# Victarry/Image-Generation-models

Measured on AMD Instinct MI355X. Metric: ddpm_cifar10_32x32_train_images_per_sec, higher is better.
Workload: dtype bf16; 1 GPU; DDPM CIFAR-10 32x32, UNet 128/1-2-4, T=1000 (BASELINE configs[1]): train step B=128/GPU + hipGraph denoise step B=64; per_gpu_batch=128, global_batch=128, parallelism=dp1, step_launch=hipGraph replay, denoise_batch=64, rccl_ranks=1, state_finite=True, matmul=bf16 MFMA, fp32 accumulate

## Files before the change

image-generation-models_amd/csrc/conv_pw.hip:

```cpp
#include "tr_common.h"

#ifndef MI_PW_PABL
#define MI_PW_PABL 0
#endif
#ifndef MI_PW_GNSABL
#define MI_PW_GNSABL 0
#endif
#ifndef MI_PW_FXABL
#define MI_PW_FXABL 0
#endif
#ifdef MI_PW_TIMING
__device__ uint32_t g_pw_ts[1024 * 4 * 5 * 64];
__device__ __forceinline__ uint32_t pw_wlane(uint32_t val, uint32_t lane, uint32_t v) {
    uint32_t keep;
    asm volatile("s_mov_b32 %1, m0\n\ts_mov_b32 m0, %3\n\ts_nop 0\n\tv_writelane_b32 %0, %2, m0\n\ts_mov_b32 m0, %1"
                 : "+v"(v), "=&s"(keep) : "s"(__builtin_amdgcn_readfirstlane(val)), "s"(__builtin_amdgcn_readfirstlane(lane)));
    return v;
}
extern "C" int mi_debug_pw_ts(uint32_t* host_out) { return (int)hipMemcpyFromSymbol(host_out, HIP_SYMBOL(g_pw_ts), sizeof(g_pw_ts)); }
#endif

namespace {

typedef uint32_t u32x2 __attribute__((ext_vector_type(2)));
// ... 1 lines not shown
__device__ __attribute__((aligned(16))) uint32_t g_zero_page3[64];

struct PwArgs {
    const uint16_t* x; const uint16_t* x2; const uint16_t* w; const float* bias; const float* res; void* y;
    int N, H, W, K, Nc, K1, ldx, ldx2, ldy, ldr, accumulate, flip;
    int TH, TI, XP, tiles_per_img, xmap;
    int qmap, gx, gy;
    uint32_t tpi_magic, cpq_magic, nch_magic, cpg_magic; int ppx, cpq, lnsub;
    const void* zero;
    float* gsum;
    const float* coef;
    const float* sums; const float* gamma; const float* beta; const float* temb;
    int ldt, cpg, hw, ng; float eps;
    double icnt;
    int ksplit; float* sk_part; int* sk_flag;
};

constexpr int pw_xp(int pt) { return pt == 256 ? 320 : pt == 128 ? 192 : 128; }

__device__ __forceinline__ int pw_fastdiv(int x, uint32_t magic) { return magic ? (int)__umulhi((uint32_t)x, magic) : x; }
inline uint32_t pw_magic(int d) { return d > 1 ? (uint32_t)((0x100000000ULL + (unsigned)d - 1) / (unsigned)d) : 0u; }

__device__ __forceinline__ void glds16s(const void* sbase, uint32_t voff, uint32_t lds_dst) {
    const uint64_t p = (uint64_t)(uintptr_t)sbase;
    const uint32_t lo = __builtin_amdgcn_readfirstlane((uint32_t)p), hi = __builtin_amdgcn_readfirstlane((uint32_t)(p >> 32));
    const uint64_t q = ((uint64_t)hi << 32) | lo;
    const uint32_t dst = __builtin_amdgcn_readfirstlane(lds_dst);
    uint32_t keep;
    asm volatile("s_mov_b32 %0, m0\n\ts_mov_b32 m0, %3\n\ts_nop 0\n\tglobal_load_lds_dwordx4 %1, %2\n\ts_mov_b32 m0, %0"
                 : "=&s"(keep) : "v"(voff), "s"(q), "s"(dst) : "memory");
// ... 31 lines not shown
    const u32x4 v = __builtin_bit_cast(u32x4, c);
    uint32_t a0, a1;
    if constexpr (DIR == 0)
        asm("v_and_b32_dpp %0, %2, %4 wave_shr:1 row_mask:0xf bank_mask:0xf bound_ctrl:1\n\t"
            "v_and_b32_dpp %1, %3, %4 wave_shr:1 row_mask:0xf bank_mask:0xf bound_ctrl:1"
            : "=&v"(a0), "=&v"(a1) : "v"(v[2 * HALF]), "v"(v[2 * HALF + 1]), "v"(mask));
    else
        asm("v_and_b32_dpp %0, %2, %4 wave_shl:1 row_mask:0xf bank_mask:0xf bound_ctrl:1\n\t"
            "v_and_b32_dpp %1, %3, %4 wave_shl:1 row_mask:0xf bank_mask:0xf bound_ctrl:1"
            : "=&v"(a0), "=&v"(a1) : "v"(v[2 * HALF]), "v"(v[2 * HALF + 1]), "v"(mask));
    o[2 * HALF] = a0; o[2 * HALF + 1] = a1;
}

constexpr int pw_lds(int pt, bool raw = false) { return (pt == 256 ? 128 : pt == 128 ? (raw ? 72 : 64) : (raw ? 48 : 32)) * 1024 + 2048; }

template <bool OUT16, int VAR = 0, int ZERO = 0, int PT = 128, bool IN32 = false, bool F32 = false>
__global__ __launch_bounds__(256, PT == 256 ? 1 : 2) void conv_pw_kernel(const PwArgs a) {
    MI_PRIO_UP();
    static_assert(ZERO == 0, "unused: kept so that the recorded kernel symbols (profiles, launch-name tests) stay valid");
#ifdef MI_PW_TIMING
    constexpr bool TIMED = VAR == 0 && !IN32 && !F32;
    uint32_t tv[5] = {0u, 0u, 0u, 0u, 0u};
    uint64_t tprev = 0;
    if constexpr (TIMED) {
        tprev = __builtin_amdgcn_s_memtime();
        tv[4] = pw_wlane((uint32_t)wall_clock64(), 7, tv[4]);
        tv[4] = pw_wlane((uint32_t)tprev, 3, tv[4]);
    }
#define MI_PW_STAMP(SET, LANE) do { if constexpr (TIMED) { tv[SET] = pw_wlane((uint32_t)tprev, (LANE), tv[SET]); tprev = __builtin_amdgcn_s_memtime(); } } while (0)
#define MI_PW_NOW(LANE) do { if constexpr (TIMED) { tv[4] = pw_wlane((uint32_t)__builtin_amdgcn_s_memtime(), (LANE), tv[4]); } } while (0)
#else
#define MI_PW_STAMP(SET, LANE) do {} while (0)
#define MI_PW_NOW(LANE) do {} while (0)
#endif
// ... 749 lines not shown
                for (int rq = 0; rq < 4; ++rq) {
                    const int ck = 8 * wv + 2 * rq + (l >> 5);
                    typedef __attribute__((address_space(3))) f32x4 lds_f32x4b;
                    const f32x4 bq = *(lds_f32x4b*)(uintptr_t)(lds0 + BIASL + 16 * ck);
#pragma unroll
                    for (int i = 0; i < BH; ++i) {
                        const int p = ep_p0 + i * a.W;
                        *(lds_u32x2*)(uintptr_t)(lds0 + p * 256 + ((ck ^ ((p & 15) << 1)) << 3)) =
                            u32x2{pack_bf16(acc[i][4 * rq] + bq.x, acc[i][4 * rq + 1] + bq.y), pack_bf16(acc[i][4 * rq + 2] + bq.z, acc[i][4 * rq + 3] + bq.w)};
                    }
                }
            }
            __syncthreads();
            MI_PW_NOW(14);
            const int j = t & 15, col = n0 + 8 * j;
            float gs[2][2] = {{0.f, 0.f}, {0.f, 0.f}};
            if (col < a.Nc) {
#pragma unroll
                for (int it = 0; it < PT / 16; ++it) {
                    const int p = it * 16 + (t >> 4);
                    const u32x4 o = *(lds_u32x4e*)(uintptr_t)(lds0 + p * 256 + (((2 * j) ^ ((p & 15) << 1)) << 3));
                    *reinterpret_cast<u32x4*>(reinterpret_cast<uint16_t*>(a.y) + ((size_t)m0 + p) * a.ldy + col) = o;
                    if constexpr (GNS && MI_PW_GNSABL != 2) {
#pragma unroll
                        for (int q = 0; q < 4; ++q) {
                            const float e0 = __uint_as_float(o[q] << 16), e1 = __uint_as_float(o[q] & 0xffff0000u);
                            gs[PT >= 256 ? 0 : it / (PT / 32)][0] += e0 + e1; gs[PT >= 256 ? 0 : it / (PT / 32)][1] += e0 * e0 + e1 * e1;
                        }
                    }
                }
// ... 819 lines not shown
        if (d->K % 128 || d->K1 % 128 || d->K1 <= 0 || d->K1 > d->K || d->Nc % 64 || d->ldx % 4 || (d->K1 != d->K && d->ldx2 % 4)) return false;
        return ((long)d->N * d->OH * d->OW) % 128 == 0;
    }
    if (f32) {
        if (d->KH != 1 || d->KW != 1 || d->pad != 0 || d->stride != 1 || d->mode != 0 || d->IH != d->OH || d->IW != d->OW) return false;
        if (d->K % 64 || d->K1 % 64 || d->K1 <= 0 || d->K1 > d->K || d->Nc % 64 || d->ldx % 4 || (d->K1 != d->K && d->ldx2 % 4)) return false;
        return ((long)d->N * d->OH * d->OW) % 128 == 0;
    }
    if (d->KH != 1 || d->KW != 1 || d->pad != 0 || d->stride != 1 || d->mode != 1) return false;
    if (d->IH != d->OH || d->IW != d->OW) return false;
    if (d->K % 128 || d->K1 % 128 || d->K1 <= 0 || d->K1 > d->K || d->Nc % 64 || d->ldx % 8 || (d->K1 != d->K && d->ldx2 % 8)) return false;
    return ((long)d->N * d->OH * d->OW) % 128 == 0;
}

struct PwGn { const float* sums; const float* gamma; const float* beta; const float* temb; int ldt, G; float eps; };

static int pw_launch(const char* who, const MiConvDesc* d, const void* x, const void* x2, const void* w_frag_bf16, const float* bias,
                     const float* residual, void* y, int out_bf16, int var, float* gsum, const float* coef, void* stream,
                     const PwGn* gn = nullptr, bool in32 = false, bool f32 = false) {
    PwArgs a{};
    if (!d || !x || !w_frag_bf16 || !y) return mi_set_error(-1, "%s: null argument", who);
    const int pt = pw_pick_tile(d, var, &a.TH, &a.TI, in32, f32, &a.ksplit);
    if (!pt) return mi_set_error(-1, "%s: descriptor not supported by the private-weight-stream conv kernel", who);
    int dev_ = 0;
    (void)hipGetDevice(&dev_);
    if (a.ksplit > 1) {
        uint8_t* ws = reinterpret_cast<uint8_t*>(g_pw_sk_ws[dev_ & 63].load(std::memory_order_acquire));
        a.sk_flag = reinterpret_cast<int*>(ws); a.sk_part = reinterpret_cast<float*>(ws + PW_SK_FLAG_BYTES);
#ifdef MI_PW_SK_ABL
        a.sk_flag = nullptr;
#endif
    }
    if (d->K1 != d->K && !x2) return mi_set_error(-1, "%s: two-source split without x2", who);
    if ((((uintptr_t)x | (uintptr_t)(x2 ? x2 : x) | (uintptr_t)w_frag_bf16) & 15) != 0) return mi_set_error(-1, "%s: operands must be 16-byte aligned", who);
    if (d->ldy % 8 || (residual && d->ldr % 4)) return mi_set_error(-1, "%s: output pixel stride must be a multiple of 8, the residual's of 4", who);
    if (var >= 2 && (a.TI != 1 || d->K1 != d->K))
        return mi_set_error(-1, "%s: the fused variants need one image per tile and one source", who);
    if (var == 2 && (!coef || ((uintptr_t)coef & 15)))
// ... 31 lines not shown
    grid.z = (unsigned)a.ksplit;
    hipStream_t st = (hipStream_t)stream;
    size_t lds = pw_lds(pt, in32 && var < 2);
    if (var >= 2) {
        const size_t need = (size_t)2 * pw_xp(pt) * 128 + 2048 + (size_t)12 * d->K;
        if (need > lds) lds = need;
    }
#define MI_PW_GO_T(O16, V, T) do { \
        static MiPerDevice once_; \
        once_.run([] { (void)hipFuncSetAttribute((const void*)conv_pw_kernel<O16, V, 0, T>, hipFuncAttributeMaxDynamicSharedMemorySize, 160 * 1024); }); \
        hipLaunchKernelGGL((conv_pw_kernel<O16, V, 0, T>), grid, dim3(256), lds, st, a); } while (0)
#define MI_PW_GO_X(O16, V, T) do { \
        static MiPerDevice once_; \
        once_.run([] { (void)hipFuncSetAttribute((const void*)conv_pw_kernel<O16, V, 0, T, true>, hipFuncAttributeMaxDynamicSharedMemorySize, 160 * 1024); }); \
        hipLaunchKernelGGL((conv_pw_kernel<O16, V, 0, T, true>), grid, dim3(256), lds, st, a); } while (0)
    if (f32) {
#define MI_PW_GO_F(T) do { \
        static MiPerDevice once_; \
        once_.run([] { (void)hipFuncSetAttribute((const void*)conv_pw_kernel<false, 0, 0, T, false, true>, hipFuncAttributeMaxDynamicSharedMemorySize, 160 * 1024); }); \
        hipLaunchKernelGGL((conv_pw_kernel<false, 0, 0, T, false, true>), grid, dim3(256), lds, st, a); } while (0)
        if (out_bf16) return mi_set_error(-1, "%s: the exact-fp32 kernel writes fp32", who);
        if (pt == 64) MI_PW_GO_F(64); else MI_PW_GO_F(128);
#undef MI_PW_GO_F
    } else if (in32) {
        if (pt == 64) switch (var) {
            case 1: if (out_bf16) MI_PW_GO_X(true, 1, 64); else MI_PW_GO_X(false, 1, 64); break;
            case 2: if (out_bf16) MI_PW_GO_X(true, 2, 64); else MI_PW_GO_X(false, 2, 64); break;
            case 3: if (out_bf16) MI_PW_GO_X(true, 3, 64); else MI_PW_GO_X(false, 3, 64); break;
            default: if (out_bf16) MI_PW_GO_X(true, 0, 64); else MI_PW_GO_X(false, 0, 64); break;
        } else switch (var) {
            case 1: if (out_bf16) MI_PW_GO_X(true, 1, 128); else MI_PW_GO_X(false, 1, 128); break;
// ... 65 lines not shown
    return (d && pw_pick_tile(d, 2, &th, &ti) && ti == 1 && d->K1 == d->K) ? 1 : 0;
}
extern "C" int mi_conv3x3_pw_gn_mish_tile(const MiConvDesc* d) {
    int th, ti;
    const int pt = d ? pw_pick_tile(d, 2, &th, &ti) : 0;
    return (pt && ti == 1 && d->K1 == d->K) ? pt : 0;
}

extern "C" int mi_conv3x3_pw(const MiConvDesc* d, const void* x, const void* x2, const void* w_frag_bf16, const float* bias,
                             const float* residual, void* y, int out_bf16, void* stream) {
    return pw_launch(__func__, d, x, x2, w_frag_bf16, bias, residual, y, out_bf16, 0, nullptr, nullptr, stream);
}
extern "C" int mi_conv3x3_pw_gnsums(const MiConvDesc* d, const void* x, const void* x2, const void* w_frag_bf16, const float* bias,
                                    const float* residual, void* y, int out_bf16, float* gsum, void* stream) {
    return pw_launch(__func__, d, x, x2, w_frag_bf16, bias, residual, y, out_bf16, 1, gsum, nullptr, stream);
}
extern "C" int mi_conv3x3_pw_x32_supported(const MiConvDesc* d) {
    int th, ti;
    return (d && pw_pick_tile(d, 0, &th, &ti, true)) ? 1 : 0;
}
extern "C" int mi_conv3x3_pw_x32_tile(const MiConvDesc* d) {
    int th, ti;
    return d ? pw_pick_tile(d, 0, &th, &ti, true) : 0;
}
extern "C" int mi_conv3x3_pw_x32(const MiConvDesc* d, const float* x, const float* x2, const void* w_frag_bf16, const float* bias,
                                 const float* residual, void* y, int out_bf16, float* gsum, void* stream) {
    return pw_launch(__func__, d, x, x2, w_frag_bf16, bias, residual, y, out_bf16, gsum ? 1 : 0, gsum, nullptr, stream, nullptr, true);
}
extern "C" int mi_conv3x3_pw_f32_tile(const MiConvDesc* d) {
    int th, ti;
// ... 341 lines not shown
```

image-generation-models_amd/src/models/ddpm.py:

```python
from __future__ import annotations

import math
import os
from functools import partial
from typing import Dict, List, Optional, Sequence, Tuple

import numpy as np
import torch
from torch import nn

from ..ops import functional as K
from .base import BaseModel, ValidationResult

_HEADS, _DHEAD = 4, 32
_GN_GROUPS = 8


def _mode_id(name: str) -> int:
    if name not in ("fp32", "bf16"):
        raise ValueError(f"compute mode must be 'fp32' or 'bf16', got {name!r}")
    return K.MODE_BF16 if name == "bf16" else K.MODE_FP32


class _Entry:
# ... 194 lines not shown
        self.compute_mode = os.environ.get("MI_DDPM_MODE", "fp32")
        self.block_storage = os.environ.get("MI_DDPM_STORAGE", "bf16")
        self.fuse_gn_conv = os.environ.get("MI_DDPM_FUSE_GN", "auto")
        self.s2_wgrad_tr = K.debug_knob("MI_DDPM_S2_TR", "1") != "0"
        self.final_block16 = K.debug_knob("MI_DDPM_FINAL16", "1") != "0"
        self.ends16 = K.debug_knob("MI_DDPM_ENDS16", "1") != "0"
        self.dual_out = K.debug_knob("MI_DDPM_DUAL_OUT", "1") != "0"
        self.fuse_ln_qkv = K.debug_knob("MI_DDPM_FUSE_LN", "1") != "0"
        self.fuse_ln_qkv_train = K.debug_knob("MI_DDPM_FUSE_LN_TRAIN", "1") != "0"
        self.small_cin_dual = K.debug_knob("MI_DDPM_CIN_DUAL", "1") != "0"
        self.cin_dual_chores = K.debug_knob("MI_DDPM_CIN_CHORES", "1") != "0"
        self.fold_attn = K.debug_knob("MI_DDPM_FOLD_ATTN", "0") == "1"
        self.small_cout_bwd1 = K.debug_knob("MI_DDPM_COUT_BWD1", "1") != "0"
        self.fuse_final = K.debug_knob("MI_DDPM_FUSE_FINAL", "1") != "0"
        self.grad_store = K.debug_knob("MI_DDPM_GRAD_STORE", "1") != "0"
        self.accumulate_grads = False
        self.grad_ready_hook = None

        flat = torch.zeros(arch.flat_numel)
        for e in arch.entries:
            if e.init == "kaiming":
                w = torch.empty(e.shape)
                nn.init.kaiming_uniform_(w, a=math.sqrt(5))
                e.logical_view(flat).copy_(w)
            elif e.init == "ubias":
                bound = 1 / math.sqrt(e.fan_in) if e.fan_in > 0 else 0
                e.logical_view(flat).copy_(torch.empty(e.shape).uniform_(-bound, bound))
            elif e.init == "one":
                e.logical_view(flat).fill_(1.0)
        object.__setattr__(self, "_flat", flat)
# ... 324 lines not shown
            elif c1_16 and eval16 and x2 is None and id(inp) in sh:
                inp_c = sh[id(inp)][1]
            tb = tb_all[:, blk["tcol"]:blk["tcol"] + co] if tb_all is not None else None
            hw = inp.shape[1] * inp.shape[2]
            fmode = str(self.fuse_gn_conv)
            sums_ok = ((co // _GN_GROUPS) % 16 == 0 and hw % 32 == 0 and ci % 32 == 0
                       and all(K.fast3x3_supported(B, inp.shape[1], inp.shape[2], ci, co, k1)))
            fuse = (not record and mode == K.MODE_BF16 and fmode != "0" and c1_16 == lo16
                    and K.conv3x3_gn_mish_supported(B, inp.shape[1], inp.shape[2], co, co))
            if fuse and fmode == "auto":
                fuse = lo16 and sums_ok and K.conv3x3_pw_gn_mish_picked(B, inp.shape[1], inp.shape[2], co, co)
            sums = None
            if fuse and fmode in ("2", "auto") and sums_ok:
                sums = take_sums(co, inp.device)
            r_pre = None
            if (blk["res"] and x2 is None and sums is None and self.small_cin_dual and K.small_cin_supported(3, ci, co)
                    and K.small_cin_dual_supported(B, inp.shape[1], inp.shape[2], ci, co, K.ld_of(inp))):
                od = BF if (c1_16 and K.small_cin_bf16_supported(3, B, inp.shape[1], inp.shape[2], ci, co, K.ld_of(inp))) else torch.float32
                if not record and mode == K.MODE_BF16 and zpool[0] is None and str(self.fuse_gn_conv) != "0" and self.cin_dual_chores:
                    zpool[0] = torch.empty(2 * B * (sum(rb["cout"] // 16 + 1 for rb in A.res_blocks) + A.dim // 16 + 1), device=inp.device, dtype=torch.int64)
                    zfill = zpool[0]
                else:
                    zfill = None
                c1, r_pre = K.conv_small_cin_fwd_dual(inp, sv[pre + "block1.block.0.weight"], sv[pre + "block1.block.0.bias"],
                                                      sv[pre + "res_conv.weight"], sv[pre + "res_conv.bias"], co, out_dtype=od, zero=zfill,
                                                      gather=tb_pending.pop() if tb_pending else None)
            else:
                c1 = conv(inp_c, pre + "block1.block.0.", 3, 1, 1, x2=x2_c, out_dtype=BF if c1_16 else torch.float32, gn_sums=sums)
            c2 = None
            if fuse:
                if sums is not None:
                    st1 = None
                    c2 = K.conv3x3_gn_mish(c1, None, wf_sh[offs[pre + "block2.block.0.weight"]:], K=co, Nc=co, bias=sv[pre + "block2.block.0.bias"],
                                           gn=(sums, sv[pre + "block1.block.1.weight"], sv[pre + "block1.block.1.bias"], tb, _GN_GROUPS, 1e-5),
                                           wq=wfq_sh[offs[pre + "block2.block.0.weight"]:])
                else:
                    st1, coef = K.gn_stats_coef(c1, sv[pre + "block1.block.1.weight"], sv[pre + "block1.block.1.bias"], temb=tb)
                    c2 = K.conv3x3_gn_mish(c1, coef, wf_sh[offs[pre + "block2.block.0.weight"]:], K=co, Nc=co, bias=sv[pre + "block2.block.0.bias"],
                                           wq=wfq_sh[offs[pre + "block2.block.0.weight"]:])
                h1 = None
            if c2 is None:
                h1, st1 = K.gn_mish_fwd(c1, sv[pre + "block1.block.1.weight"], sv[pre + "block1.block.1.bias"], temb=tb,
                                        out_dtype=BF if lo16 else torch.float32)
                c2 = conv(h1, pre + "block2.block.0.", 3, 1, 1, out_dtype=BF if lo16 else torch.float32)
            r = inp
            if r_pre is not None:
                r = r_pre
            elif blk["res"]:
                r = None
                if inp_c is not inp and inp_c.dtype == BF and (x2 is None or x2_c is not None):
                    r = conv(inp_c, pre + "res_conv.", 1, x2=x2_c, soft=True)
                if r is None:
                    r = conv(inp, pre + "res_conv.", 1, x2=x2)
            if want_out16 and (use_sh or (eval16 and out16_in_eval)) and co % 32 == 0:
                out, st2, out16 = K.gn_mish_fwd(c2, sv[pre + "block2.block.1.weight"], sv[pre + "block2.block.1.bias"], residual=r, want16=True)
                sh[id(out)] = (out, out16)
            else:
                out, st2 = K.gn_mish_fwd(c2, sv[pre + "block2.block.1.weight"], sv[pre + "block2.block.1.bias"], residual=r)
            if record:
                tape.append(("res", blk, inp, x2, c1, st1, h1, c2, st2, out, inp_c, x2_c))
            return out

        def attention(at, inp, feeds_s2=False):
            pre = at["pre"]
            c = inp.shape[3]
            a16 = (mode == K.MODE_BF16 and self.block_storage in ("bf16", "auto") and B % 8 == 0
                   and all(K.fast1x1_supported(B, inp.shape[1], inp.shape[2], c, 3 * _HEADS * _DHEAD))
                   and all(K.fast1x1_supported(B, inp.shape[1], inp.shape[2], _HEADS * _DHEAD, c)))
            dt = BF if a16 else torch.float32
# ... 586 lines not shown
```

image-generation-models_amd/src/ops/functional.py:

```python
from __future__ import annotations

import ctypes as C
import functools
import os
from typing import Optional, Tuple

import torch

from .lib import ROWSUM_MAX, WGRAD_STORE, MiConvDesc, MiGnDesc, MiRowSum, MiWgradDesc, check, load_library

MODE_FP32, MODE_BF16 = 0, 1


def debug_knob(name: str, default: str) -> str:
    if os.environ.get("MI_DEBUG_KNOBS") == "1":
        return os.environ.get(name, default)
    return default
PROBE = None


CONV_AUTO = os.environ.get("MI_CONV_AUTO", "1") == "1"


USE_CONV_PW = CONV_AUTO and debug_knob("MI_CONV_PW", "1") == "1"
# ... 314 lines not shown
              "mi_conv3x3_bf16w_io")
    else:
        check(lib.mi_conv3x3_bf16w(C.byref(d), _p(x), _p(x2), _p(wsh), _p(bias), _p(residual), _p(out), _stream()),
              "mi_conv3x3_bf16w")
    if e0 is not None:
        bm, ck, sk = C.c_int(), C.c_int(), C.c_int()
        lib.mi_conv3x3_bf16w_tile(C.byref(d), io, C.byref(bm), C.byref(ck), C.byref(sk))
        nb = (N * H * W * K * _esz(x) + N * H * W * Nc * (_esz(out) * (2 if accumulate else 1) + _esz(residual))
              + ksize * ksize * K * Nc * 2)
        _probe_close(e0, f"conv3x3_halo_kernel<{bm.value}, {ck.value}, {ksize}, {'true' if sk.value else 'false'}, {io}, {8 if bm.value == 256 or (bm.value == 128 and ck.value == 64) else 4}>",
                     2.0 * N * H * W * Nc * K * ksize * ksize,
                     f"N{N} {H}x{W} K{K}{'(2src)' if x2 is not None else ''}->{Nc} flip{int(flip)} acc{int(accumulate)} io{io}", nb)
    return (out, y16) if want16 else out


def gn_stats_coef(x, gamma, beta, *, groups=8, eps=1e-5, temb=None):
    _need_gpu(x)
    N, H, W, Cc = x.shape
    stats = torch.empty((N, groups, 2), device=x.device, dtype=torch.float32)
    coef = torch.empty((3, N, Cc), device=x.device, dtype=torch.float32)
    d = MiGnDesc(N=N, HW=H * W, C=Cc, G=groups, eps=eps, ldx=ld_of(x), ldy=Cc, ldr=0)
    e0 = _probe_open()
    check(load_library().mi_gn_stats_coef(C.byref(d), _p(x), _p(gamma), _p(beta), _p(temb), ld_of(temb) if temb is not None else 0,
                                          _p(stats), _p(coef), _b16(x), _stream()), "mi_gn_stats_coef")
    if e0 is not None:
        _probe_close(e0, f"gn_mish_fwd_kernel<io{_b16(x)}> (statistics only)", 0.0, f"N{N} HW{H * W} C{Cc}", N * H * W * Cc * _esz(x))
    return stats, coef


GSUM_SCALE = float(1 << 20)
# ... 1691 lines not shown
```

image-generation-models_amd/src/ops/lib.py:

```python
from __future__ import annotations

import ctypes as C
import os

_PKG_ROOT = os.path.dirname(os.path.dirname(os.path.dirname(os.path.abspath(__file__))))
_LIB = None


def library_path() -> str:
    return os.environ.get("MI_DDPM_LIB", os.path.join(_PKG_ROOT, "lib", "libmi_ddpm.so"))


class MiConvDesc(C.Structure):
    _fields_ = [(n, C.c_int) for n in (
        "N", "IH", "IW", "OH", "OW", "K", "Nc", "KH", "KW", "stride", "pad", "transposed", "w_kn", "mode",
        "K1", "ldx", "ldx2", "ldy", "ldr", "accumulate")]


class MiWgradDesc(C.Structure):
    _fields_ = [(n, C.c_int) for n in (
        "N", "GH", "GW", "DH", "DW", "Ci", "Cj", "KH", "KW", "stride", "pad", "gather_i", "mode", "I1",
        "ldp", "ldp2", "ldq")]


# ... 88 lines not shown
    "mi_debug_conv_pw_splitk": [_I],
    "mi_ln_conv1x1_pw_supported": [C.POINTER(MiConvDesc)],
    "mi_ln_conv1x1_pw": [C.POINTER(MiConvDesc), _P, _P, _P, C.c_float, _P, _P, _P, _P],
    "mi_ln_conv1x1_pw_dual": [C.POINTER(MiConvDesc), _P, _P, _P, C.c_float, _P, _P, _P, _P, _I, _P],
    "mi_conv1x1_pw_f32_supported": [C.POINTER(MiConvDesc)],
    "mi_conv1x1_pw_f32": [C.POINTER(MiConvDesc), _P, _P, _P, _P, _P, _P, _P],
    "mi_pack_weights_f32frag": [_I, _P, _I, _P, _P, _P, _P],
    "mi_conv3x3_pw_x32_supported": [C.POINTER(MiConvDesc)],
    "mi_conv3x3_pw_x32_tile": [C.POINTER(MiConvDesc)],
    "mi_conv3x3_pw_x32": [C.POINTER(MiConvDesc), _P, _P, _P, _P, _P, _P, _I, _P, _P],
    "mi_conv3x3_pw": [C.POINTER(MiConvDesc), _P, _P, _P, _P, _P, _P, _I, _P],
    "mi_conv3x3_pw_gn_mish_supported": [C.POINTER(MiConvDesc)],
    "mi_conv1x1_pw_supported": [C.POINTER(MiConvDesc)],
    "mi_conv1x1_pw": [C.POINTER(MiConvDesc), _P, _P, _P, _P, _P, _P, _I, _P, _I, _P],
    "mi_conv3x3_pw_gnsums": [C.POINTER(MiConvDesc), _P, _P, _P, _P, _P, _P, _I, _P, _P],
    "mi_conv3x3_pw_gn_mish": [C.POINTER(MiConvDesc), _P, _P, _P, _P, _P, _I, _P],
    "mi_conv3x3_pw_gn_mish_sums": [C.POINTER(MiConvDesc), _P, _P, _P, _P, _P, _I, _I, _F, _P, _P, _P, _I, _P],
    "mi_conv3x3_pw_x32_gn_mish_supported": [C.POINTER(MiConvDesc)],
    "mi_conv3x3_pw_x32_gn_mish_tile": [C.POINTER(MiConvDesc)],
    "mi_conv3x3_pw_gn_mish_tile": [C.POINTER(MiConvDesc)],
    "mi_conv3x3_pw_x32_gn_mish": [C.POINTER(MiConvDesc), _P, _P, _P, _P, _P, _I, _P],
    "mi_conv3x3_pw_x32_gn_mish_sums": [C.POINTER(MiConvDesc), _P, _P, _P, _P, _P, _I, _I, _F, _P, _P, _P, _I, _P],
    "mi_gn_stats_coef": [C.POINTER(MiGnDesc), _P, _P, _P, _P, _I, _P, _P, _I, _P],
    "mi_conv3x3_gn_mish_supported": [C.POINTER(MiConvDesc)],
    "mi_conv3x3_gn_mish_tile": [C.POINTER(MiConvDesc), C.POINTER(C.c_int), C.POINTER(C.c_int)],
    "mi_conv3x3_gn_mish": [C.POINTER(MiConvDesc), _P, _P, _P, _P, _P, _I, _P],
    "mi_conv3x3_small_cin_fwd": [_I, _I, _I, _I, _I, _P, _I, _P, _P, _P, _I, _P],
    "mi_conv3x3_small_cin_wgrad": [_I, _I, _I, _I, _I, _P, _I, _P, _I, _P, _P],
    "mi_conv1x1_small_cout": [_I, _I, _I, _I, _P, _I, _P, _I, _P, _P, _P, _I, _I, _P],
    "mi_conv1x1_small_cout_ws": [_I, _I, _I, _I, _P, _I, _P, _I, _P, _P, _P, _I, _I, _P, _Z, _P],
# ... 172 lines not shown
```

include/mi_ddpm.h:

```cpp
#ifndef MI_DDPM_H
#define MI_DDPM_H
#include <stddef.h>
#include <stdint.h>

#ifdef __cplusplus
extern "C" {
#endif

#define MI_ABI_VERSION 4
#define MI_MODE_FP32 0
#define MI_MODE_BF16 1

int mi_abi_version(void);
const char* mi_last_error(void);

typedef struct MiConvDesc {
    int N;
    int IH, IW;
    int OH, OW;
    int K;
    int Nc;
    int KH, KW, stride, pad;
    int transposed;
    int w_kn;
// ... 63 lines not shown
int mi_ln_conv1x1_pw_dual(const MiConvDesc* d, const float* x, const float* ln_g, const float* ln_b, float eps, const void* w_frag_bf16,
                          const float* bias, void* y_bf16, void* ln_bf16, int ldl, void* stream);
int mi_conv1x1_pw_f32_supported(const MiConvDesc* d);
int mi_conv1x1_pw_f32(const MiConvDesc* d, const float* x, const float* x2, const float* w_frag_f32, const float* bias,
                      const float* residual, float* y, void* stream);
int mi_pack_weights_f32frag(int nent, const void* entries_dev, int total_tiles, const float* master, float* wdq32, float* wfq32,
                            void* stream);
int mi_debug_conv_pw_tile(int pt);
int mi_debug_conv_pw_auto256(int min_workgroups);
int mi_debug_conv1x1_pw_nloop(int on);
int mi_conv3x3_pw_tile(const MiConvDesc* d);
int mi_conv3x3_pw(const MiConvDesc* d, const void* x, const void* x2, const void* w_frag_bf16, const float* bias,
                  const float* residual, void* y, int out_bf16, void* stream);
int mi_conv3x3_pw_gnsums(const MiConvDesc* d, const void* x, const void* x2, const void* w_frag_bf16, const float* bias,
                         const float* residual, void* y, int out_bf16, float* gsum, void* stream);
int mi_conv3x3_pw_gn_mish_supported(const MiConvDesc* d);
int mi_conv3x3_pw_gn_mish_tile(const MiConvDesc* d);
int mi_conv3x3_pw_gn_mish(const MiConvDesc* d, const void* x, const float* coef, const void* w_frag_bf16, const float* bias,
                          void* y, int out_bf16, void* stream);
int mi_conv3x3_pw_gn_mish_sums(const MiConvDesc* d, const void* x, const float* sums, const float* gamma, const float* beta,
                               const float* temb, int ldt, int G, float eps, const void* w_frag_bf16, const float* bias,
                               void* y, int out_bf16, void* stream);
int mi_conv3x3_pw_x32_gn_mish_supported(const MiConvDesc* d);
int mi_conv3x3_pw_x32_gn_mish_tile(const MiConvDesc* d);
int mi_conv3x3_pw_x32_gn_mish(const MiConvDesc* d, const float* x, const float* coef, const void* w_frag_bf16, const float* bias,
                              void* y, int out_bf16, void* stream);
int mi_conv3x3_pw_x32_gn_mish_sums(const MiConvDesc* d, const float* x, const float* sums, const float* gamma, const float* beta,
                                   const float* temb, int ldt, int G, float eps, const void* w_frag_bf16, const float* bias,
                                   void* y, int out_bf16, void* stream);
int mi_conv1x1_pw_supported(const MiConvDesc* d);
// ... 350 lines not shown
```

Before: 27120 images/s.

## Fuse GroupNorm+Mish(+temb/residual) epilogue into 3x3 conv for 8x8 resblocks

Result: no change. 27270 images/s (median of 6 runs) (+0.5%).

```diff
diff --git a/image-generation-models_amd/csrc/conv_pw.hip b/image-generation-models_amd/csrc/conv_pw.hip
--- a/image-generation-models_amd/csrc/conv_pw.hip
+++ b/image-generation-models_amd/csrc/conv_pw.hip
@@ -39,6 +39,7 @@
     int ldt, cpg, hw, ng; float eps;
     double icnt;
     int ksplit; float* sk_part; int* sk_flag;
+    float* gn_stats; void* gn_h; uint16_t* gn_h16; const float* gn_res; int gn_ldh, gn_ldh16, gn_ldr;
 };
 
 constexpr int pw_xp(int pt) { return pt == 256 ? 320 : pt == 128 ? 192 : 128; }
@@ -100,10 +101,10 @@
 
 constexpr int pw_lds(int pt, bool raw = false) { return (pt == 256 ? 128 : pt == 128 ? (raw ? 72 : 64) : (raw ? 48 : 32)) * 1024 + 2048; }
 
-template <bool OUT16, int VAR = 0, int ZERO = 0, int PT = 128, bool IN32 = false, bool F32 = false>
+template <bool OUT16, int VAR = 0, int GNE = 0, int PT = 128, bool IN32 = false, bool F32 = false>
 __global__ __launch_bounds__(256, PT == 256 ? 1 : 2) void conv_pw_kernel(const PwArgs a) {
     MI_PRIO_UP();
-    static_assert(ZERO == 0, "unused: kept so that the recorded kernel symbols (profiles, launch-name tests) stay valid");
+    static_assert(GNE == 0 || (GNE <= 2 && OUT16 && VAR == 0 && PT <= 128 && !IN32 && !F32), "GroupNorm epilogue: the plain bf16 conv, whole 8x8 images per tile");
 #ifdef MI_PW_TIMING
     constexpr bool TIMED = VAR == 0 && !IN32 && !F32;
     uint32_t tv[5] = {0u, 0u, 0u, 0u, 0u};
@@ -883,6 +884,110 @@
             __syncthreads();
             MI_PW_NOW(14);
             const int j = t & 15, col = n0 + 8 * j;
+            if constexpr (GNE != 0) {
+                constexpr int NS = PT / 64, NU = NS * 4;
+                const int pr = t >> 4, smp0 = m0 >> 6, lcpg = 31 - __builtin_clz(a.cpg);
+                f32x4 rr[GNE == 2 ? NU : 1][2];
+                if constexpr (GNE == 2) {
+#pragma unroll
+                    for (int u = 0; u < NU; ++u) {
+                        const float* rp = a.gn_res + ((size_t)m0 + u * 16 + pr) * a.gn_ldr + col;
+                        rr[u][0] = *reinterpret_cast<const f32x4*>(rp); rr[u][1] = *reinterpret_cast<const f32x4*>(rp + 4);
+                    }
+                }
+                f32x4 gq[2], bq[2], tq[NS][2];
+#pragma unroll
+                for (int h = 0; h < 2; ++h) {
+                    gq[h] = *reinterpret_cast<const f32x4*>(a.gamma + col + 4 * h); bq[h] = *reinterpret_cast<const f32x4*>(a.beta + col + 4 * h);
+#pragma unroll
+                    for (int s = 0; s < NS; ++s)
+                        tq[s][h] = a.temb ? *reinterpret_cast<const f32x4*>(a.temb + (size_t)(smp0 + s) * a.ldt + col + 4 * h) : f32x4{0.f, 0.f, 0.f, 0.f};
+                }
+                u32x4 o[NU];
+#pragma unroll
+                for (int u = 0; u < NU; ++u) {
+                    const int p = u * 16 + pr;
+                    o[u] = *(lds_u32x4e*)(uintptr_t)(lds0 + p * 256 + (((2 * j) ^ ((p & 15) << 1)) << 3));
+                    *reinterpret_cast<u32x4*>(reinterpret_cast<uint16_t*>(a.y) + ((size_t)m0 + p) * a.ldy + col) = o[u];
+                }
+                auto el = [&](int u, int e) -> float { const uint32_t v = o[u][e >> 1]; return __uint_as_float((e & 1) ? (v & 0xffff0000u) : (v << 16)); };
+                float* red = reinterpret_cast<float*>(lds_raw + DUMP);
+                auto slice_sum = [&](float (&v)[NS], int slot) {
+#pragma unroll
+                    for (int s = 0; s < NS; ++s) {
+                        float r = v[s];
+                        r += __shfl_xor(r, 1, 64);
+                        if (a.cpg >= 32) r += __shfl_xor(r, 2, 64);
+                        if (a.cpg >= 64) r += __shfl_xor(r, 4, 64);
+                        r += __shfl_xor(r, 16, 64); r += __shfl_xor(r, 32, 64);
+                        if (l < 16) red[((slot * 4 + wv) * NS + s) * 16 + l] = r;
+                    }
+                    asm volatile("s_waitcnt lgkmcnt(0)" ::: "memory");
+                    __builtin_amdgcn_s_barrier();
+                    asm volatile("" ::: "memory");
+#pragma unroll
+                    for (int s = 0; s < NS; ++s)
+                        v[s] = ((red[((slot * 4 + 0) * NS + s) * 16 + j] + red[((slot * 4 + 1) * NS + s) * 16 + j])
+                                + red[((slot * 4 + 2) * NS + s) * 16 + j]) + red[((slot * 4 + 3) * NS + s) * 16 + j];
+                };
+                const float cnt = 64.f * (float)a.cpg;
+                float mean[NS], rstd[NS];
+#pragma unroll
+                for (int s = 0; s < NS; ++s) {
+                    float sm = 0.f;
+#pragma unroll
+                    for (int k = 0; k < 4; ++k)
+#pragma unroll
+                        for (int e = 0; e < 8; ++e) sm += el(s * 4 + k, e);
+                    mean[s] = sm;
+                }
+                slice_sum(mean, 0);
+#pragma unroll
+                for (int s = 0; s < NS; ++s) {
+                    mean[s] = mean[s] / cnt;
+                    float s2 = 0.f;
+#pragma unroll
+                    for (int k = 0; k < 4; ++k)
+#pragma unroll
+                        for (int e = 0; e < 8; ++e) { const float dlt = el(s * 4 + k, e) - mean[s]; s2 += dlt * dlt; }
+                    rstd[s] = s2;
+                }
+                slice_sum(rstd, 1);
+#pragma unroll
+                for (int s = 0; s < NS; ++s) {
+                    rstd[s] = 1.0f / sqrtf(rstd[s] / cnt + a.eps);
+                    if (pr == 0 && (col & (a.cpg - 1)) == 0) {
+                        float* sp = a.gn_stats + ((size_t)(smp0 + s) * a.ng + (col >> lcpg)) * 2;
+                        sp[0] = mean[s]; sp[1] = rstd[s];
+                    }
+                    float ga[8], be[8];
+#pragma unroll
+                    for (int e = 0; e < 8; ++e) { ga[e] = gq[e >> 2][e & 3] * rstd[s]; be[e] = bq[e >> 2][e & 3] - mean[s] * ga[e]; }
+#pragma unroll
+                    for (int k = 0; k < 4; ++k) {
+                        const int u = s * 4 + k;
+                        const size_t m = (size_t)m0 + u * 16 + pr;
+                        float hv[8];
+#pragma unroll
+                        for (int e = 0; e < 8; ++e) {
+                            hv[e] = mish_fast_f(el(u, e) * ga[e] + be[e]) + tq[s][e >> 2][e & 3];
+                            if constexpr (GNE == 2) hv[e] += rr[u][e >> 2][e & 3];
+                        }
+                        const u32x4 h16 = {pack_bf16(hv[0], hv[1]), pack_bf16(hv[2], hv[3]), pack_bf16(hv[4], hv[5]), pack_bf16(hv[6], hv[7])};
+                        if constexpr (GNE == 1) {
+                            *reinterpret_cast<u32x4*>(reinterpret_cast<uint16_t*>(a.gn_h) + m * a.gn_ldh + col) = h16;
+                        } else {
+                            float* yp = reinterpret_cast<float*>(a.gn_h) + m * a.gn_ldh + col;
+                            *reinterpret_cast<f32x4*>(yp) = f32x4{hv[0], hv[1], hv[2], hv[3]};
+                            *reinterpret_cast<f32x4*>(yp + 4) = f32x4{hv[4], hv[5], hv[6], hv[7]};
+                            if (a.gn_h16) *reinterpret_cast<u32x4*>(a.gn_h16 + m * a.gn_ldh16 + col) = h16;
+                        }
+                    }
+                }
+                MI_PW_NOW(15);
+                ts_out();
+                return;
+            }
             float gs[2][2] = {{0.f, 0.f}, {0.f, 0.f}};
             if (col < a.Nc) {
 #pragma unroll
@@ -1732,14 +1837,34 @@
 }
 
 struct PwGn { const float* sums; const float* gamma; const float* beta; const float* temb; int ldt, G; float eps; };
+struct PwGnEp { int form; const float* gamma; const float* beta; const float* temb; int ldt, G; float eps; float* stats; void* h; int ldh;
+                const float* res; int ldr; void* h16; int ldh16; };
+
+bool pw_gn_ep_ok(const MiConvDesc* d, int G, int pt, int TH) {
+    if (!pt || pt > 128 || d->mode != 1 || d->OH != 8 || d->OW != 8 || TH != d->OH || d->accumulate || d->transposed) return false;
+    if (G <= 0 || d->Nc % 128 || d->Nc % G) return false;
+    const int cpg = d->Nc / G;
+    return cpg == 16 || cpg == 32 || cpg == 64;
+}
 
 static int pw_launch(const char* who, const MiConvDesc* d, const void* x, const void* x2, const void* w_frag_bf16, const float* bias,
                      const float* residual, void* y, int out_bf16, int var, float* gsum, const float* coef, void* stream,
-                     const PwGn* gn = nullptr, bool in32 = false, bool f32 = false) {
+                     const PwGn* gn = nullptr, bool in32 = false, bool f32 = false, const PwGnEp* ep = nullptr) {
     PwArgs a{};
     if (!d || !x || !w_frag_bf16 || !y) return mi_set_error(-1, "%s: null argument", who);
     const int pt = pw_pick_tile(d, var, &a.TH, &a.TI, in32, f32, &a.ksplit);
+    if (ep && !pw_gn_ep_ok(d, ep->G, (var == 0 && !in32 && !f32 && out_bf16 && !residual) ? pt : 0, a.TH)) return 1;
     if (!pt) return mi_set_error(-1, "%s: descriptor not supported by the private-weight-stream conv kernel", who);
+    if (ep) {
+        if ((ep->form != 1 && ep->form != 2) || !ep->gamma || !ep->beta || !ep->stats || !ep->h || (ep->form == 2 && !ep->res))
+            return mi_set_error(-1, "%s: form 1 or 2; gamma, beta, stats, h (form 2: the residual)", who);
+        if ((((uintptr_t)ep->gamma | (uintptr_t)ep->beta | (uintptr_t)ep->h | (uintptr_t)ep->h16 | (uintptr_t)ep->res | (uintptr_t)ep->temb) & 15) || ((uintptr_t)ep->stats & 3)
+            || ep->ldh % (ep->form == 1 ? 8 : 4) || (ep->temb && ep->ldt % 4) || (ep->res && ep->ldr % 4) || (ep->h16 && ep->ldh16 % 8) || (ep->form == 1 && (ep->res || ep->h16)))
+            return mi_set_error(-1, "%s: misaligned GroupNorm epilogue operands", who);
+        a.gamma = ep->gamma; a.beta = ep->beta; a.temb = ep->temb; a.ldt = ep->ldt; a.ng = ep->G; a.cpg = d->Nc / ep->G; a.eps = ep->eps;
+        a.gn_stats = ep->stats; a.gn_h = ep->h; a.gn_ldh = ep->ldh; a.gn_res = ep->res; a.gn_ldr = ep->ldr;
+        a.gn_h16 = reinterpret_cast<uint16_t*>(ep->h16); a.gn_ldh16 = ep->ldh16;
+    }
     int dev_ = 0;
     (void)hipGetDevice(&dev_);
     if (a.ksplit > 1) {
@@ -1801,7 +1926,15 @@
         static MiPerDevice once_; \
         once_.run([] { (void)hipFuncSetAttribute((const void*)conv_pw_kernel<O16, V, 0, T, true>, hipFuncAttributeMaxDynamicSharedMemorySize, 160 * 1024); }); \
         hipLaunchKernelGGL((conv_pw_kernel<O16, V, 0, T, true>), grid, dim3(256), lds, st, a); } while (0)
-    if (f32) {
+    if (ep) {
+#define MI_PW_GO_E(E, T) do { \
+        static MiPerDevice once_; \
+        once_.run([] { (void)hipFuncSetAttribute((const void*)conv_pw_kernel<true, 0, E, T>, hipFuncAttributeMaxDynamicSharedMemorySize, 160 * 1024); }); \
+        hipLaunchKernelGGL((conv_pw_kernel<true, 0, E, T>), grid, dim3(256), lds, st, a); } while (0)
+        if (ep->form == 1) { if (pt == 64) MI_PW_GO_E(1, 64); else MI_PW_GO_E(1, 128); }
+        else { if (pt == 64) MI_PW_GO_E(2, 64); else MI_PW_GO_E(2, 128); }
+#undef MI_PW_GO_E
+    } else if (f32) {
 #define MI_PW_GO_F(T) do { \
         static MiPerDevice once_; \
         once_.run([] { (void)hipFuncSetAttribute((const void*)conv_pw_kernel<false, 0, 0, T, false, true>, hipFuncAttributeMaxDynamicSharedMemorySize, 160 * 1024); }); \
@@ -1897,6 +2030,17 @@
 extern "C" int mi_conv3x3_pw_gnsums(const MiConvDesc* d, const void* x, const void* x2, const void* w_frag_bf16, const float* bias,
                                     const float* residual, void* y, int out_bf16, float* gsum, void* stream) {
     return pw_launch(__func__, d, x, x2, w_frag_bf16, bias, residual, y, out_bf16, 1, gsum, nullptr, stream);
+}
+extern "C" int mi_conv3x3_pw_gn_epilogue_supported(const MiConvDesc* d, int G) {
+    int th = 0, ti = 0, ks = 1;
+    const int pt = d ? pw_pick_tile(d, 0, &th, &ti, false, false, &ks) : 0;
+    return (pt && pw_gn_ep_ok(d, G, pt, th)) ? 1 : 0;
+}
+extern "C" int mi_conv3x3_pw_gn_epilogue(const MiConvDesc* d, const void* x, const void* x2, const void* w_frag_bf16, const float* bias, void* c,
+                                         int form, const float* gamma, const float* beta, int G, float eps, const float* temb, int ldt,
+                                         float* stats, void* h, int ldh, const float* res, int ldr, void* h16, int ldh16, void* stream) {
+    const PwGnEp ep{form, gamma, beta, temb, ldt, G, eps, stats, h, ldh, res, ldr, h16, ldh16};
+    return pw_launch(__func__, d, x, x2, w_frag_bf16, bias, nullptr, c, 1, 0, nullptr, nullptr, stream, nullptr, false, false, &ep);
 }
 extern "C" int mi_conv3x3_pw_x32_supported(const MiConvDesc* d) {
     int th, ti;
diff --git a/image-generation-models_amd/src/models/ddpm.py b/image-generation-models_amd/src/models/ddpm.py
--- a/image-generation-models_amd/src/models/ddpm.py
+++ b/image-generation-models_amd/src/models/ddpm.py
@@ -232,6 +232,7 @@
         self.small_cout_bwd1 = K.debug_knob("MI_DDPM_COUT_BWD1", "1") != "0"
         self.fuse_final = K.debug_knob("MI_DDPM_FUSE_FINAL", "1") != "0"
         self.grad_store = K.debug_knob("MI_DDPM_GRAD_STORE", "1") != "0"
+        self.gn_epilogue = "auto" if K.debug_knob("MI_DDPM_GN_EPILOGUE", "auto") != "0" else False
         self.accumulate_grads = False
         self.grad_ready_hook = None
 
@@ -586,6 +587,9 @@
             if fuse and fmode in ("2", "auto") and sums_ok:
                 sums = take_sums(co, inp.device)
             r_pre = None
+            gne = (record and self.gn_epilogue and mode == K.MODE_BF16 and lo16
+                   and K.conv3x3_gn_epilogue_supported(B, inp.shape[1], inp.shape[2], co, co, groups=_GN_GROUPS))
+            ep1 = ep2 = None
             if (blk["res"] and x2 is None and sums is None and self.small_cin_dual and K.small_cin_supported(3, ci, co)
                     and K.small_cin_dual_supported(B, inp.shape[1], inp.shape[2], ci, co, K.ld_of(inp))):
                 od = BF if (c1_16 and K.small_cin_bf16_supported(3, B, inp.shape[1], inp.shape[2], ci, co, K.ld_of(inp))) else torch.float32
@@ -598,7 +602,14 @@
                                                       sv[pre + "res_conv.weight"], sv[pre + "res_conv.bias"], co, out_dtype=od, zero=zfill,
                                                       gather=tb_pending.pop() if tb_pending else None)
             else:
-                c1 = conv(inp_c, pre + "block1.block.0.", 3, 1, 1, x2=x2_c, out_dtype=BF if c1_16 else torch.float32, gn_sums=sums)
+                if gne and c1_16 and inp_c.dtype == BF and (x2 is None or x2_c is not None):
+                    ep1 = K.conv3x3_gn_epilogue(inp_c, wfq_sh[offs[pre + "block1.block.0.weight"]:], sv[pre + "block1.block.1.weight"],
+                                                sv[pre + "block1.block.1.bias"], K=ci, Nc=co, x2=x2_c, bias=sv[pre + "block1.block.0.bias"],
+                                                groups=_GN_GROUPS, temb=tb)
+                if ep1 is None:
+                    c1 = conv(inp_c, pre + "block1.block.0.", 3, 1, 1, x2=x2_c, out_dtype=BF if c1_16 else torch.float32, gn_sums=sums)
+                else:
+                    c1, st1, h1 = ep1
             c2 = None
             if fuse:
                 if sums is not None:
@@ -611,20 +622,42 @@
                     c2 = K.conv3x3_gn_mish(c1, coef, wf_sh[offs[pre + "block2.block.0.weight"]:], K=co, Nc=co, bias=sv[pre + "block2.block.0.bias"],
                                            wq=wfq_sh[offs[pre + "block2.block.0.weight"]:])
                 h1 = None
-            if c2 is None:
+            if c2 is None and ep1 is None:
                 h1, st1 = K.gn_mish_fwd(c1, sv[pre + "block1.block.1.weight"], sv[pre + "block1.block.1.bias"], temb=tb,
                                         out_dtype=BF if lo16 else torch.float32)
+            w16 = bool(want_out16 and (use_sh or (eval16 and out16_in_eval)) and co % 32 == 0)
+
+            def res_input():
+                r = inp
+                if r_pre is not None:
+                    r = r_pre
+                elif blk["res"]:
+                    r = None
+                    if inp_c is not inp and inp_c.dtype == BF and (x2 is None or x2_c is not None):
+                        r = conv(inp_c, pre + "res_conv.", 1, x2=x2_c, soft=True)
+                    if r is None:
+                        r = conv(inp, pre + "res_conv.", 1, x2=x2)
+                return r
+
+            r = None
+            if c2 is None and gne and h1 is not None and h1.dtype == BF:
+                r = res_input()
+                if r.dtype == torch.float32:
+                    ep2 = K.conv3x3_gn_epilogue(h1, wfq_sh[offs[pre + "block2.block.0.weight"]:], sv[pre + "block2.block.1.weight"],
+                                                sv[pre + "block2.block.1.bias"], K=co, Nc=co, bias=sv[pre + "block2.block.0.bias"],
+                                                groups=_GN_GROUPS, residual=r, want16=w16)
+            if ep2 is not None:
+                c2, st2, out = ep2[:3]
+                if w16:
+                    sh[id(out)] = (out, ep2[3])
+                if record:
+                    tape.append(("res", blk, inp, x2, c1, st1, h1, c2, st2, out, inp_c, x2_c))
+                return out
+            if c2 is None:
                 c2 = conv(h1, pre + "block2.block.0.", 3, 1, 1, out_dtype=BF if lo16 else torch.float32)
-            r = inp
-            if r_pre is not None:
-                r = r_pre
-            elif blk["res"]:
-                r = None
-                if inp_c is not inp and inp_c.dtype == BF and (x2 is None or x2_c is not None):
-                    r = conv(inp_c, pre + "res_conv.", 1, x2=x2_c, soft=True)
-                if r is None:
-                    r = conv(inp, pre + "res_conv.", 1, x2=x2)
-            if want_out16 and (use_sh or (eval16 and out16_in_eval)) and co % 32 == 0:
+            if r is None:
+                r = res_input()
+            if w16:
                 out, st2, out16 = K.gn_mish_fwd(c2, sv[pre + "block2.block.1.weight"], sv[pre + "block2.block.1.bias"], residual=r, want16=True)
                 sh[id(out)] = (out, out16)
             else:
diff --git a/image-generation-models_amd/src/ops/functional.py b/image-generation-models_amd/src/ops/functional.py
--- a/image-generation-models_amd/src/ops/functional.py
+++ b/image-generation-models_amd/src/ops/functional.py
@@ -352,6 +352,50 @@
     return (out, y16) if want16 else out
 
 
+def _gn_ep_desc(N, H, W, K, Nc, K1, ldx, ldx2, ldy):
+    return MiConvDesc(N=N, IH=H, IW=W, OH=H, OW=W, K=K, Nc=Nc, KH=3, KW=3, stride=1, pad=1, transposed=0, w_kn=0, mode=MODE_BF16,
+                      K1=K1, ldx=ldx, ldx2=ldx2, ldy=ldy, ldr=0, accumulate=0)
+
+
+def conv3x3_gn_epilogue_supported(N, H, W, K, Nc, K1=None, groups=8, mode=MODE_BF16):
+    if mode != MODE_BF16 or not USE_CONV_PW:
+        return False
+    d = _gn_ep_desc(N, H, W, K, Nc, K if K1 is None else K1, K if K1 is None else K1, K - K1 if K1 is not None else 0, Nc)
+    return bool(_pick_pw(N, H, W, K, Nc, d) and _query("mi_conv3x3_pw_gn_epilogue_supported", d, groups))
+
+
+def conv3x3_gn_epilogue(x, wq, gamma, beta, *, K, Nc, x2=None, bias=None, groups=8, eps=1e-5, temb=None, residual=None, want16=False):
+    _need_gpu(x)
+    N, H, W, K1 = x.shape
+    if x2 is None:
+        K1 = K
+    if x.dtype != torch.bfloat16 or (x2 is not None and x2.dtype != torch.bfloat16) or wq is None or not USE_CONV_PW:
+        return None
+    d = _gn_ep_desc(N, H, W, K, Nc, K1, ld_of(x), ld_of(x2) if x2 is not None else 0, Nc)
+    if not (_pick_pw(N, H, W, K, Nc, d) and _query("mi_conv3x3_pw_gn_epilogue_supported", d, groups)):
+        return None
+    form = 1 if residual is None else 2
+    assert form == 2 or not want16
+    c = new_act(N, H, W, Nc, x, torch.bfloat16)
+    h = new_act(N, H, W, Nc, x, torch.bfloat16 if form == 1 else torch.float32)
+    h16 = new_act(N, H, W, Nc, x, torch.bfloat16) if want16 else None
+    stats = torch.empty((N, groups, 2), device=x.device, dtype=torch.float32)
+    e0 = _probe_open()
+    rc = load_library().mi_conv3x3_pw_gn_epilogue(
+        C.byref(d), _p(x), _p(x2), _p(wq), _p(bias), _p(c), form, _p(gamma), _p(beta), groups, eps, _p(temb),
+        ld_of(temb) if temb is not None else 0, _p(stats), _p(h), ld_of(h), _p(residual), ld_of(residual) if residual is not None else 0,
+        _p(h16), ld_of(h16) if h16 is not None else 0, _stream())
+    if rc == 1:
+        raise RuntimeError("mi_conv3x3_pw_gn_epilogue refused a descriptor its _supported query accepted")
+    check(rc, "mi_conv3x3_pw_gn_epilogue")
+    if e0 is not None:
+        nb = (N * H * W * K * 2 + N * H * W * Nc * (2 + _esz(h) + _esz(residual) + (2 if want16 else 0)) + 9 * K * Nc * 2)
+        pt = _pw_tile_now(d, 0, False, _query("mi_conv3x3_pw_tile", d))
+        _probe_close(e0, f"conv_pw_kernel<true, 0, {form}, {pt or 128}>", 2.0 * N * H * W * Nc * K * 9,
+                     f"N{N} {H}x{W} K{K}{'(2src)' if x2 is not None else ''}->{Nc} + GroupNorm epilogue form {form}", nb)
+    return (c, stats, h, h16) if want16 else (c, stats, h)
+
+
 def gn_stats_coef(x, gamma, beta, *, groups=8, eps=1e-5, temb=None):
     _need_gpu(x)
     N, H, W, Cc = x.shape
diff --git a/image-generation-models_amd/src/ops/lib.py b/image-generation-models_amd/src/ops/lib.py
--- a/image-generation-models_amd/src/ops/lib.py
+++ b/image-generation-models_amd/src/ops/lib.py
@@ -126,6 +126,8 @@
     "mi_conv1x1_pw_supported": [C.POINTER(MiConvDesc)],
     "mi_conv1x1_pw": [C.POINTER(MiConvDesc), _P, _P, _P, _P, _P, _P, _I, _P, _I, _P],
     "mi_conv3x3_pw_gnsums": [C.POINTER(MiConvDesc), _P, _P, _P, _P, _P, _P, _I, _P, _P],
+    "mi_conv3x3_pw_gn_epilogue_supported": [C.POINTER(MiConvDesc), _I],
+    "mi_conv3x3_pw_gn_epilogue": [C.POINTER(MiConvDesc), _P, _P, _P, _P, _P, _I, _P, _P, _I, _F, _P, _I, _P, _P, _I, _P, _I, _P, _I, _P],
     "mi_conv3x3_pw_gn_mish": [C.POINTER(MiConvDesc), _P, _P, _P, _P, _P, _I, _P],
     "mi_conv3x3_pw_gn_mish_sums": [C.POINTER(MiConvDesc), _P, _P, _P, _P, _P, _I, _I, _F, _P, _P, _P, _I, _P],
     "mi_conv3x3_pw_x32_gn_mish_supported": [C.POINTER(MiConvDesc)],
diff --git a/include/mi_ddpm.h b/include/mi_ddpm.h
--- a/include/mi_ddpm.h
+++ b/include/mi_ddpm.h
@@ -101,6 +101,10 @@
                   const float* residual, void* y, int out_bf16, void* stream);
 int mi_conv3x3_pw_gnsums(const MiConvDesc* d, const void* x, const void* x2, const void* w_frag_bf16, const float* bias,
                          const float* residual, void* y, int out_bf16, float* gsum, void* stream);
+int mi_conv3x3_pw_gn_epilogue_supported(const MiConvDesc* d, int G);
+int mi_conv3x3_pw_gn_epilogue(const MiConvDesc* d, const void* x, const void* x2, const void* w_frag_bf16, const float* bias, void* c,
+                              int form, const float* gamma, const float* beta, int G, float eps, const float* temb, int ldt,
+                              float* stats, void* h, int ldh, const float* res, int ldr, void* h16, int ldh16, void* stream);
 int mi_conv3x3_pw_gn_mish_supported(const MiConvDesc* d);
 int mi_conv3x3_pw_gn_mish_tile(const MiConvDesc* d);
 int mi_conv3x3_pw_gn_mish(const MiConvDesc* d, const void* x, const float* coef, const void* w_frag_bf16, const float* bias,
```
